# splinterhq/libsplinter

Measured on AMD Instinct MI355X. Metric: KV set/get ops/sec + Nomic-768d embed vectors/sec at 1/2/4/8 MI355X, higher is better.
Workload: dtype bf16

## Files before the change

libsplinter_amd/csrc/hip/gemm384.hip:

```cpp
#include <hip/hip_runtime.h>
#include <cstdint>
#include <cstdlib>

#include "gemm_tile.hpp"
#include "nomic_api.h"

namespace {

typedef __bf16 bf16x8 __attribute__((ext_vector_type(8)));
typedef __bf16 bf16x2_t __attribute__((ext_vector_type(2)));
typedef float f32x4 __attribute__((ext_vector_type(4)));
typedef __attribute__((address_space(3))) void lds_void;
typedef const __attribute__((address_space(1))) void gbl_void;

constexpr int kBM = spl::kGemm384BM;
constexpr int kBN = spl::kGemm384BN;
constexpr int kBK = 32;
constexpr int kWN = kBN / 2;
constexpr int kNT = kWN / 16;
constexpr int kThreads = 512;
constexpr int kRowBytes = kBK * 2;
constexpr int kABytes = kBM * kRowBytes;
constexpr int kWBytes = kBN * kRowBytes;

__device__ __forceinline__ uint32_t pk2(float a, float b) {
  const bf16x2_t v = {(__bf16)a, (__bf16)b};
  return __builtin_bit_cast(uint32_t, v);
}

__device__ __forceinline__ void raw_barrier() {
  asm volatile("" ::: "memory");
  __builtin_amdgcn_s_barrier();
  asm volatile("" ::: "memory");
}

__device__ __forceinline__ void wait_vm(int n) {
  switch (n) {
    case 3: asm volatile("s_waitcnt vmcnt(3)" ::: "memory"); break;
    default: asm volatile("s_waitcnt vmcnt(0)" ::: "memory"); break;
  }
}

__device__ __forceinline__ uint32_t xor16(uint32_t v) { return (uint32_t)__builtin_amdgcn_ds_swizzle((int)v, 0x401F); }

__device__ __forceinline__ int swz(int r, int c) { return c ^ ((r >> 1) & 3); }

__device__ __forceinline__ void rotate(float a, float b, float c, float s, bool plain, float& x1, float& x2) {
  float p1, p2;
  {
#pragma clang fp contract(off)
    p1 = a * c - b * s;
    p2 = b * c + a * s;
  }
  float bs, as;
  {
#pragma clang fp contract(off)
    bs = b * s;
    as = a * s;
  }
  const float f1 = __builtin_fmaf(a, c, -bs), f2 = __builtin_fmaf(b, c, as);
  x1 = plain ? p1 : f1;
  x2 = plain ? p2 : f2;
}

struct Epi384 {
  uint16_t* out;
  long ldo;
  const float* rope;
  const int32_t* pos;
  int rope_cols;
  long M;
  int gn;
};

constexpr int kNW = 3, kNA = 2;
constexpr int kLdsBytes = kNW * kWBytes + kNA * kABytes;
static_assert(kLdsBytes <= 160 * 1024, "LDS budget");

template <int MODE>
__global__ __launch_bounds__(kThreads, 1) void k_gemm384(const uint16_t* __restrict__ A, long lda,
                                                         const uint16_t* __restrict__ W, long ldw, int K,
                                                         int mtiles, int ntiles, Epi384 ep) {
  constexpr int LW = kNW - 1, LA = kNA - 1;
  static_assert(LW > LA, "an iteration issues its A stage before its W stage");
  constexpr int kABase = kNW * kWBytes;
  constexpr int kWaves = kThreads / 64;
  constexpr int RW = kBM / 4, MT = RW / 16;
  constexpr int GA = kBM / 16 / kWaves, GW = kBN / 16 / kWaves;
  static_assert(GA == 2 && GW == 3 && MT == 4, "wait_vm's cases and the epilogues assume this split");
  static_assert(MODE == NOMIC_EPI_STORE || MODE == NOMIC_EPI_SWIGLU || MODE == NOMIC_EPI_ROPE, "epilogues");
  extern __shared__ __attribute__((aligned(16))) char smem[];
  const int tid = threadIdx.x, lane = tid & 63, wave = tid >> 6;
  const int wr = wave >> 1, wn = wave & 1;
  int mt, nt;
  spl::remap_tile(blockIdx.x, mtiles * ntiles, ntiles, ep.gn, mt, nt);
  const long m0 = (long)mt * kBM, n0 = (long)nt * kBN;
  A += m0 * lda;
  W += n0 * ldw;

  const int drow = lane >> 2, dpc = lane & 3;
  uint32_t offA[GA];
#pragma unroll
  for (int i = 0; i < GA; ++i) {
    const int r = (wave + kWaves * i) * 16 + drow;
    const long gr = (m0 + r < ep.M) ? r : ep.M - 1 - m0;
    offA[i] = (uint32_t)(gr * lda + swz(r, dpc) * 8);
  }
  uint32_t offW[GW];
#pragma unroll
  for (int i = 0; i < GW; ++i) {
    const int r = (wave + kWaves * i) * 16 + drow;
    offW[i] = (uint32_t)(r * ldw + swz(r, dpc) * 8);
  }
  const int nk = K / kBK;
  auto glds_w = [&](int t, int i) {
    __builtin_amdgcn_global_load_lds((gbl_void*)(W + (long)t * kBK + offW[i]),
                                     (lds_void*)(smem + (t % kNW) * kWBytes + (wave + kWaves * i) * 1024), 16, 0, 0);
  };
  auto glds_a = [&](int t, int i) {
    __builtin_amdgcn_global_load_lds((gbl_void*)(A + (long)t * kBK + offA[i]),
                                     (lds_void*)(smem + kABase + (t % kNA) * kABytes + (wave + kWaves * i) * 1024),
                                     16, 0, 0);
  };
  constexpr int kOps = GA + GW;
  static_assert(kOps <= kNT, "two DMAs ahead of each of the kNT / 2 MFMA pairs cover a stage's loads");
  auto issue_op = [&](int s, int u) {
    const int tw = s + LW, ta = s + LA;
    if (u < GA) { if (ta >= 0 && ta < nk) glds_a(ta, u); }
    else if (tw >= 0 && tw < nk) glds_w(tw, u - GA);
  };
  auto issue = [&](int s) {
#pragma unroll
    for (int u = 0; u < kOps; ++u) issue_op(s, u);
  };
  auto younger = [&](int t) -> int { return t + LW - 1 < nk ? GW : 0; };

  const int fl = (lane & 15) * kRowBytes + (swz(lane & 15, lane >> 4) << 4);
  const int aoff = kABase + (wr * RW) * kRowBytes + fl;
  const int woff = (wn * kWN) * kRowBytes + fl;

  f32x4 acc[MT][kNT];
#pragma unroll
  for (int i = 0; i < MT; ++i)
#pragma unroll
    for (int j = 0; j < kNT; ++j) acc[i][j] = f32x4{0.f, 0.f, 0.f, 0.f};
  for (int s = -LW; s < 0; ++s) issue(s);
  for (int t = 0; t < nk; ++t) {
    wait_vm(younger(t));
    raw_barrier();
    const char* bw = smem + (t % kNW) * kWBytes;
    const char* ba = smem + (t % kNA) * kABytes;
    bf16x8 af[MT], w0, w1, x0, x1;
#pragma unroll
    for (int i = 0; i < MT; ++i) af[i] = *(const bf16x8*)(ba + aoff + i * 16 * kRowBytes);
    w0 = *(const bf16x8*)(bw + woff);
    w1 = *(const bf16x8*)(bw + woff + 16 * kRowBytes);
    __builtin_amdgcn_s_setprio(1);
#pragma unroll
    for (int jp = 0; jp < kNT / 2; ++jp) {
#pragma unroll
      for (int u = 2 * jp; u < 2 * jp + 2; ++u)
        if (u < kOps) issue_op(t, u);
      if (jp + 1 < kNT / 2) {
        x0 = *(const bf16x8*)(bw + woff + (2 * (jp + 1)) * 16 * kRowBytes);
        x1 = *(const bf16x8*)(bw + woff + (2 * (jp + 1) + 1) * 16 * kRowBytes);
      }
#pragma unroll
      for (int i = 0; i < MT; ++i) {
        acc[i][2 * jp] = __builtin_amdgcn_mfma_f32_16x16x32_bf16(w0, af[i], acc[i][2 * jp], 0, 0, 0);
        acc[i][2 * jp + 1] = __builtin_amdgcn_mfma_f32_16x16x32_bf16(w1, af[i], acc[i][2 * jp + 1], 0, 0, 0);
      }
      __builtin_amdgcn_sched_barrier(0);
      w0 = x0;
      w1 = x1;
    }
    __builtin_amdgcn_s_setprio(0);
  }

  const int rl = lane & 15, cq = (lane >> 4) * 4;
  const bool odd = (lane >> 4) & 1;
  const int h8 = (lane >> 5) * 8;
  const long mb = m0 + wr * RW + rl;
  auto exchange = [&](const uint32_t (&x)[2], const uint32_t (&y)[2]) -> uint4 {
    const uint32_t gx = xor16(odd ? x[0] : y[0]), gy = xor16(odd ? x[1] : y[1]);
    return odd ? make_uint4(gx, gy, y[0], y[1]) : make_uint4(x[0], x[1], gx, gy);
  };
  if constexpr (MODE == NOMIC_EPI_STORE) {
    uint16_t* o = ep.out + n0 + wn * kWN + (odd ? 16 : 0) + h8;
#pragma unroll
    for (int p = 0; p < kNT / 2; ++p)
#pragma unroll
      for (int i = 0; i < MT; ++i) {
        const long m = mb + 16 * i;
        const uint32_t x[2] = {pk2(acc[i][2 * p][0], acc[i][2 * p][1]), pk2(acc[i][2 * p][2], acc[i][2 * p][3])};
        const uint32_t y[2] = {pk2(acc[i][2 * p + 1][0], acc[i][2 * p + 1][1]),
                               pk2(acc[i][2 * p + 1][2], acc[i][2 * p + 1][3])};
        const uint4 v = exchange(x, y);
        if (m < ep.M) *(uint4*)(o + m * ep.ldo + 32 * p) = v;
      }
  } else if constexpr (MODE == NOMIC_EPI_SWIGLU) {
    uint16_t* o = ep.out + (n0 + wn * kWN) / 2 + (odd ? 16 : 0) + h8;
#pragma unroll
    for (int q = 0; q < kNT / 4; ++q)
#pragma unroll
      for (int i = 0; i < MT; ++i) {
        const long m = mb + 16 * i;
        uint32_t hk[2][2];
#pragma unroll
        for (int h = 0; h < 2; ++h) {
          const int p = 2 * q + h;
          float v[4];
#pragma unroll
          for (int e = 0; e < 4; ++e) v[e] = spl::swiglu(acc[i][2 * p][e], acc[i][2 * p + 1][e]);
          hk[h][0] = pk2(v[0], v[1]);
          hk[h][1] = pk2(v[2], v[3]);
        }
        const uint4 v = exchange(hk[0], hk[1]);
        if (m < ep.M) *(uint4*)(o + m * ep.ldo + 32 * q) = v;
      }
  } else {
#pragma unroll
    for (int i = 0; i < MT; ++i) {
      const long m = mb + 16 * i;
      const long mr = m < ep.M ? m : ep.M - 1;
      const bool rot = n0 + wn * kWN < ep.rope_cols;
      const float* cs0 = ep.rope + (rot ? (long)ep.pos[mr] * 64 : 0) + cq * 2;
#pragma unroll
      for (int half = 0; half < 2; ++half) {
        float4 ca = {}, cb = {};
        if (rot) ca = *(const float4*)(cs0 + half * 32), cb = *(const float4*)(cs0 + half * 32 + 4);
        const float cs[8] = {ca.x, ca.y, ca.z, ca.w, cb.x, cb.y, cb.z, cb.w};
#pragma unroll
        for (int head = 0; head < kWN / 64; ++head) {
          const int p = 2 * head + half;
          const long gcol = n0 + wn * kWN + head * 64;
          float x1[4], x2[4];
#pragma unroll
          for (int e = 0; e < 4; ++e) {
            x1[e] = acc[i][2 * p][e];
            x2[e] = acc[i][2 * p + 1][e];
          }
          if (gcol < ep.rope_cols) {
#pragma unroll
            for (int e = 0; e < 4; ++e) {
              rotate(x1[e], x2[e], cs[2 * e], cs[2 * e + 1], e >= 2 && odd, x1[e], x2[e]);
            }
          }
          const uint32_t x[2] = {pk2(x1[0], x1[1]), pk2(x1[2], x1[3])};
          const uint32_t y[2] = {pk2(x2[0], x2[1]), pk2(x2[2], x2[3])};
          const uint4 v = exchange(x, y);
          if (m < ep.M) *(uint4*)(ep.out + m * ep.ldo + gcol + (odd ? 32 : 0) + half * 16 + h8) = v;
        }
      }
    }
  }
}

template <int MODE>
int launch384(const uint16_t* A, long lda, const uint16_t* W, long ldw, long M, int N, int K, const Epi384& ep,
              hipStream_t s) {
  static bool attr = [] {
    (void)hipFuncSetAttribute((const void*)k_gemm384<MODE>, hipFuncAttributeMaxDynamicSharedMemorySize, kLdsBytes);
    return true;
  }();
  (void)attr;
  const int mtiles = (int)((M + kBM - 1) / kBM), ntiles = N / kBN;
  hipLaunchKernelGGL(k_gemm384<MODE>, dim3(mtiles * ntiles), dim3(kThreads), kLdsBytes, s, A, lda, W, ldw, K, mtiles,
                     ntiles, ep);
  return (int)hipGetLastError();
}

}

namespace spl {

bool gemm384_ok(int mode, const void* out, long ldo, long lda, long ldw, long M, int N, int K, const float* rope) {
  if (mode != NOMIC_EPI_STORE && mode != NOMIC_EPI_SWIGLU && mode != NOMIC_EPI_ROPE) return false;
  if (M <= 0 || N <= 0 || N % kBN || K % kBK || K < 2 * kBK) return false;
  if (lda % 8 || ldw % 8 || ldo % 8 || (uintptr_t)out % 16 || lda < K || ldw < K) return false;
  if (mode == NOMIC_EPI_ROPE && (uintptr_t)rope % 16) return false;
  const long mtiles = (M + kBM - 1) / kBM;
  return (long)kBM * lda < (1L << 31) && (long)kBN * ldw < (1L << 31) && mtiles * (N / kBN) < (1L << 31);
}

int gemm384_launch(int mode, const uint16_t* A, long lda, const uint16_t* W, long ldw, long M, int N, int K,
                   uint16_t* out, long ldo, const float* rope, const int32_t* pos, int rope_cols, int gn,
                   hipStream_t s) {
  const Epi384 ep{out, ldo, rope, pos, rope_cols, M, gn};
  switch (mode) {
    case NOMIC_EPI_STORE: return launch384<NOMIC_EPI_STORE>(A, lda, W, ldw, M, N, K, ep, s);
    case NOMIC_EPI_SWIGLU: return launch384<NOMIC_EPI_SWIGLU>(A, lda, W, ldw, M, N, K, ep, s);
    case NOMIC_EPI_ROPE: return launch384<NOMIC_EPI_ROPE>(A, lda, W, ldw, M, N, K, ep, s);
    default: return (int)hipErrorInvalidValue;
  }
}

}
```

libsplinter_amd/csrc/include/nomic_api.h:

```cpp
#ifndef SPLINTER_NOMIC_API_H
#define SPLINTER_NOMIC_API_H
#include <stdint.h>
#include "arena_api.h"

#ifdef __cplusplus
extern "C" {
#endif

#define NOMIC_EPI_STORE    0
#define NOMIC_EPI_RESIDUAL 1
#define NOMIC_EPI_SWIGLU   2
#define NOMIC_EPI_ROPE     3
#define NOMIC_EPI_F32      4
#define NOMIC_EPI_ROPE_FOLD    5
#define NOMIC_EPI_SWIGLU_FOLD  6
#define NOMIC_EPI_RES_STATS    7
#define NOMIC_EPI_RES_LN_STATS 8

int nomic_gemm(int mode, const void *A, long lda, const void *W, long ldw, long M, int N, int K,
               void *out, long ldo, const void *res, long ldr, const float *rope, const int32_t *pos,
               int rope_cols, hipStream_t stream);
int nomic_gemm_ln(int mode, const void *A, long lda, const void *W, long ldw, long M, int N, int K, void *out,
                  long ldo, const void *res, long ldr, const float *rope, const int32_t *pos, int rope_cols,
                  const float *part_in, int nparts, float eps, const float *c1, const float *c2,
                  const void *ln_g, const void *ln_b, float *part, hipStream_t stream);
int nomic_row_stats(const float *part, int nparts, long M, float eps, float *st, hipStream_t stream);
int nomic_gemm_set_variant(int variant);
int nomic_gemm_set_tail_split(int on);
long nomic_gemm256_grid(long M, int N);

int nomic_embed_ln(const int32_t *ids, long T, const void *tok_emb, const void *type_row,
                   const void *gamma, const void *beta, float eps, void *out, hipStream_t stream);
int nomic_layernorm(const void *x, long T, const void *gamma, const void *beta, float eps, void *out,
                    hipStream_t stream);
int nomic_attention_set_variant(int variant);
int nomic_attention(const void *qkv, void *out, const int32_t *cu_seqlens, const int32_t *qblocks,
                    int nqb, int heads, float scale, hipStream_t stream);
int nomic_mean_pool(const void *x, const int32_t *cu_seqlens, int B, float *pooled, int normalize,
                    spl_arena_t arena, const int64_t *slots, const uint64_t *hashes, int32_t *status,
                    hipStream_t stream);
int nomic_dequant(int ggml_type, const void *src, long nelems, void *dst_bf16, hipStream_t stream);

#ifdef __cplusplus
}
#endif
#endif
```

libsplinter_amd/models/nomic.py:

```python
from __future__ import annotations

import ctypes
import math
import os
from dataclasses import dataclass
from typing import Dict, List, Optional, Sequence, Tuple

import numpy as np
import torch

from .. import _native as N
from ..utils.tracing import trace_range
from .gguf import DEVICE_DEQUANT, GGUFFile, GGUFWriter, dequant_host

EPI_STORE, EPI_RESIDUAL, EPI_SWIGLU, EPI_ROPE, EPI_F32 = 0, 1, 2, 3, 4
EPI_ROPE_FOLD, EPI_SWIGLU_FOLD, EPI_RES_STATS, EPI_RES_LN_STATS = 5, 6, 7, 8


@dataclass
class NomicConfig:
    vocab: int = 30528
    d: int = 768
    layers: int = 12
    heads: int = 12
    ffn: int = 3072
    eps: float = 1e-12
    rope_base: float = 1000.0
    n_ctx: int = 2048
    type_vocab: int = 2

    @property
    def head_dim(self) -> int:
        return self.d // self.heads

    @classmethod
    def from_gguf(cls, g: GGUFFile) -> "NomicConfig":
        a = g.arch() or "nomic-bert"
        get = lambda k, d: g.get(f"{a}.{k}", d)
        tok = g.tensors.get("token_embd.weight")
        return cls(vocab=tok.shape[0] if tok else 30528, d=int(get("embedding_length", 768)),
                   layers=int(get("block_count", 12)), heads=int(get("attention.head_count", 12)),
                   ffn=int(get("feed_forward_length", 3072)), eps=float(get("attention.layer_norm_epsilon", 1e-12)),
                   rope_base=float(get("rope.freq_base", 1000.0)), n_ctx=int(get("context_length", 2048)))


def _lib():
    L = N.hip_lib()
    if not getattr(L, "_nomic_declared", False):
        P, c_long, c_int, c_float = ctypes.c_void_p, ctypes.c_long, ctypes.c_int, ctypes.c_float
        L.nomic_gemm.argtypes = [c_int, P, c_long, P, c_long, c_long, c_int, c_int, P, c_long, P, c_long, P, P, c_int, P]
        L.nomic_gemm.restype = c_int
        L.nomic_gemm_ln.argtypes = [c_int, P, c_long, P, c_long, c_long, c_int, c_int, P, c_long, P, c_long, P, P,
                                    c_int, P, c_int, c_float, P, P, P, P, P, P]
        L.nomic_gemm_ln.restype = c_int
        L.nomic_gemm_res_ln.argtypes = [P, c_long, P, c_long, c_long, c_int, c_int, P, c_long, P, P, c_float, P,
                                        c_long, P]
        L.nomic_gemm_res_ln.restype = c_int
        L.nomic_gemm_res_ln_set_variant.argtypes = [c_int]
        L.nomic_gemm_res_ln_set_variant.restype = c_int
        L.nomic_row_stats.argtypes = [P, c_int, c_long, c_float, P, P]
        L.nomic_row_stats.restype = c_int
        L.nomic_gemm_set_variant.argtypes = [c_int]
        L.nomic_gemm_set_variant.restype = c_int
        L.nomic_gemm_set_tail_split.argtypes = [c_int]
        L.nomic_gemm_set_tail_split.restype = c_int
        L.nomic_gemm256_grid.argtypes = [c_long, c_int]
        L.nomic_gemm256_grid.restype = c_long
        L.nomic_attention_set_variant.argtypes = [c_int]
        L.nomic_attention_set_variant.restype = c_int
        L.nomic_embed_ln.argtypes = [P, c_long, P, P, P, P, c_float, P, P]
        L.nomic_embed_ln.restype = c_int
        L.nomic_layernorm.argtypes = [P, c_long, P, P, c_float, P, P]
        L.nomic_layernorm.restype = c_int
        L.nomic_attention.argtypes = [P, P, P, P, c_int, c_int, c_float, P]
        L.nomic_attention.restype = c_int
        L.nomic_mean_pool.argtypes = [P, P, c_int, P, c_int, N.Arena, P, P, P, P]
        L.nomic_mean_pool.restype = c_int
        L.nomic_dequant.argtypes = [c_int, P, c_long, P, P]
        L.nomic_dequant.restype = c_int
        L._nomic_declared = True
    return L


def _chk(rc, what):
    if rc != 0:
        raise RuntimeError(f"{what}: HIP launch failed ({rc})")


def _stream():
    return torch.cuda.current_stream().cuda_stream


GGUF_NAMES = {
    "tok": "token_embd.weight", "type": "token_types.weight",
    "emb_g": "token_embd_norm.weight", "emb_b": "token_embd_norm.bias",
}
LAYER_NAMES = {
    "wqkv": "attn_qkv.weight", "wo": "attn_output.weight",
    "ln1_g": "attn_output_norm.weight", "ln1_b": "attn_output_norm.bias",
    "wup": "ffn_up.weight", "wgate": "ffn_gate.weight", "wdown": "ffn_down.weight",
    "ln2_g": "layer_output_norm.weight", "ln2_b": "layer_output_norm.bias",
}


def random_weights(cfg: NomicConfig, seed: int = 0, std: float = 0.02) -> Dict[str, np.ndarray]:
    rng = np.random.default_rng(seed)
    f = lambda *s: (rng.standard_normal(s) * std).astype(np.float32)
    w = {GGUF_NAMES["tok"]: f(cfg.vocab, cfg.d), GGUF_NAMES["type"]: f(cfg.type_vocab, cfg.d),
         GGUF_NAMES["emb_g"]: (1 + f(cfg.d) * 5).astype(np.float32), GGUF_NAMES["emb_b"]: f(cfg.d)}
    for i in range(cfg.layers):
        p = f"blk.{i}."
        w[p + "attn_qkv.weight"] = f(3 * cfg.d, cfg.d)
        w[p + "attn_output.weight"] = f(cfg.d, cfg.d)
        w[p + "attn_output_norm.weight"] = (1 + f(cfg.d) * 5).astype(np.float32)
        w[p + "attn_output_norm.bias"] = f(cfg.d)
        w[p + "ffn_up.weight"] = f(cfg.ffn, cfg.d)
        w[p + "ffn_gate.weight"] = f(cfg.ffn, cfg.d)
        w[p + "ffn_down.weight"] = f(cfg.d, cfg.ffn)
        w[p + "layer_output_norm.weight"] = (1 + f(cfg.d) * 5).astype(np.float32)
        w[p + "layer_output_norm.bias"] = f(cfg.d)
    return w


def write_gguf(path: str, cfg: NomicConfig, weights: Dict[str, np.ndarray], vocab: Optional[List[str]] = None,
               linear_type: str = "F16") -> None:
    w = GGUFWriter(path, "nomic-bert")
    a = "nomic-bert"
    w.add("general.name", "nomic-embed-text-v1.5 (random init)")
    w.add(f"{a}.context_length", cfg.n_ctx)
    w.add(f"{a}.embedding_length", cfg.d)
    w.add(f"{a}.feed_forward_length", cfg.ffn)
    w.add(f"{a}.attention.head_count", cfg.heads)
    w.add(f"{a}.attention.layer_norm_epsilon", float(cfg.eps))
    w.add(f"{a}.block_count", cfg.layers)
    w.add(f"{a}.rope.freq_base", float(cfg.rope_base))
    w.add(f"{a}.attention.causal", False)
    w.add(f"{a}.pooling_type", 1)
    if vocab is not None:
        w.add("tokenizer.ggml.model", "bert")
        w.add("tokenizer.ggml.tokens", vocab)
        w.add("tokenizer.ggml.token_type", [1] * len(vocab))
        ids = {t: i for i, t in enumerate(vocab)}
        for key, tok in (("bos", "[CLS]"), ("eos", "[SEP]"), ("seperator", "[SEP]"), ("unknown", "[UNK]"),
                         ("padding", "[PAD]")):
            if tok in ids:
                w.add(f"tokenizer.ggml.{key}_token_id", ids[tok])
    for name, arr in weights.items():
        lin = arr.ndim == 2 and not name.startswith("token_")
        w.add_tensor(name, arr, linear_type if lin else ("F16" if name == "token_embd.weight" else "F32"))
    w.write()


def pack_upgate(up: torch.Tensor, gate: torch.Tensor) -> torch.Tensor:
    F, d = up.shape
    return torch.stack([up.reshape(F // 16, 16, d), gate.reshape(F // 16, 16, d)], 1).reshape(2 * F, d)


_QKV_PERM = torch.cat([torch.arange(0, 16), torch.arange(32, 48), torch.arange(16, 32), torch.arange(48, 64)])


def pack_qkv(w: torch.Tensor) -> torch.Tensor:
    n, d = w.shape
    return w.reshape(n // 64, 64, d)[:, _QKV_PERM.to(w.device)].reshape(n, d)


def fold_ln(w: torch.Tensor, g: torch.Tensor, b: torch.Tensor):
    wf = (w.float() * g.float()[None, :]).to(torch.bfloat16).contiguous()
    c1 = wf.float().sum(1).contiguous()
    c2 = (w.float() @ b.float()).contiguous()
    return wf, c1, c2


class NomicWeights:

    def __init__(self, cfg: NomicConfig, tensors: Dict[str, torch.Tensor], device="cuda"):
        self.cfg = cfg
        bf = lambda t: t.to(device=device, dtype=torch.bfloat16).contiguous()
        self.tok = bf(tensors[GGUF_NAMES["tok"]])
        self.type_row = bf(tensors[GGUF_NAMES["type"]][0])
        self.emb_g, self.emb_b = bf(tensors[GGUF_NAMES["emb_g"]]), bf(tensors[GGUF_NAMES["emb_b"]])
        self.layers = []
        for i in range(cfg.layers):
            p = f"blk.{i}."
            t = {k: tensors[p + v] for k, v in LAYER_NAMES.items()}
            self.layers.append({
                "wqkv": bf(pack_qkv(t["wqkv"])), "wo": bf(t["wo"]), "wupgate": bf(pack_upgate(t["wup"], t["wgate"])),
                "wdown": bf(t["wdown"]),
                "ln1_g": bf(t["ln1_g"]), "ln1_b": bf(t["ln1_b"]), "ln2_g": bf(t["ln2_g"]), "ln2_b": bf(t["ln2_b"]),
            })
        for i, lw in enumerate(self.layers):
            lw["wupgate_f"], lw["ug_c1"], lw["ug_c2"] = fold_ln(lw["wupgate"], lw["ln1_g"], lw["ln1_b"])
            if i > 0:
                prev = self.layers[i - 1]
                lw["wqkv_f"], lw["qkv_c1"], lw["qkv_c2"] = fold_ln(lw["wqkv"], prev["ln2_g"], prev["ln2_b"])

    @classmethod
    def from_numpy(cls, cfg, weights: Dict[str, np.ndarray], device="cuda"):
        return cls(cfg, {k: torch.from_numpy(v) for k, v in weights.items()}, device)

    @classmethod
    def from_gguf(cls, g: GGUFFile, cfg: Optional[NomicConfig] = None, device="cuda"):
        cfg = cfg or NomicConfig.from_gguf(g)
        L = _lib()
        out = {}
        for name, info in g.tensors.items():
            if info.ggml_type in DEVICE_DEQUANT:
                raw = torch.from_numpy(np.ascontiguousarray(g.raw(name))).to(device)
                dst = torch.empty(info.nelems, dtype=torch.bfloat16, device=device)
                _chk(L.nomic_dequant(info.ggml_type, raw.data_ptr(), info.nelems, dst.data_ptr(), _stream()),
                     f"dequant {name}")
                out[name] = dst.view(info.shape)
            else:
                out[name] = torch.from_numpy(dequant_host(g.raw(name), info.ggml_type, info.nelems)
                                             .reshape(info.shape)).to(device)
        return cls(cfg, out, device)


class NomicReference(torch.nn.Module):

    def __init__(self, cfg: NomicConfig, weights: Dict[str, np.ndarray], device="cpu"):
        super().__init__()
        self.cfg = cfg
        self.w = {k: torch.from_numpy(np.asarray(v, np.float32)).to(device) for k, v in weights.items()}

    def rope(self, x, pos):
        hd = self.cfg.head_dim
        inv = self.cfg.rope_base ** (-torch.arange(0, hd, 2, dtype=torch.float64, device=x.device) / hd)
        ang = pos[:, None].double() * inv[None, :]
        c, s = torch.cos(ang).float()[:, None, :], torch.sin(ang).float()[:, None, :]
        x1, x2 = x[..., : hd // 2], x[..., hd // 2:]
        return torch.cat([x1 * c - x2 * s, x2 * c + x1 * s], dim=-1)

    def forward(self, ids: torch.Tensor, cu: Sequence[int]) -> torch.Tensor:
        cfg, w = self.cfg, self.w
        F = torch.nn.functional
        x = w["token_embd.weight"][ids] + w["token_types.weight"][0]
        x = F.layer_norm(x, (cfg.d,), w["token_embd_norm.weight"], w["token_embd_norm.bias"], cfg.eps)
        pos = torch.cat([torch.arange(cu[i + 1] - cu[i]) for i in range(len(cu) - 1)]).to(ids.device)
        H, hd = cfg.heads, cfg.head_dim
        for i in range(cfg.layers):
            p = f"blk.{i}."
            qkv = x @ w[p + "attn_qkv.weight"].T
            q, k, v = qkv.split(cfg.d, dim=1)
            q = self.rope(q.view(-1, H, hd), pos)
            k = self.rope(k.view(-1, H, hd), pos)
            v = v.view(-1, H, hd)
            outs = []
            for s in range(len(cu) - 1):
                a, b = cu[s], cu[s + 1]
                att = torch.einsum("qhd,khd->hqk", q[a:b], k[a:b]) / math.sqrt(hd)
                outs.append(torch.einsum("hqk,khd->qhd", att.softmax(-1), v[a:b]))
            o = torch.cat(outs).reshape(-1, cfg.d)
            x = F.layer_norm(o @ w[p + "attn_output.weight"].T + x, (cfg.d,), w[p + "attn_output_norm.weight"],
                             w[p + "attn_output_norm.bias"], cfg.eps)
            up = x @ w[p + "ffn_up.weight"].T
            gate = x @ w[p + "ffn_gate.weight"].T
            h = (up * F.silu(gate)) @ w[p + "ffn_down.weight"].T
            x = F.layer_norm(h + x, (cfg.d,), w[p + "layer_output_norm.weight"], w[p + "layer_output_norm.bias"],
                             cfg.eps)
        return torch.stack([x[cu[s]: cu[s + 1]].mean(0) for s in range(len(cu) - 1)])


class Batch:

    def __init__(self, seqs: Sequence[Sequence[int]], device="cuda", qblock: int = 128):
        lens = [len(s) for s in seqs]
        assert all(n > 0 for n in lens), "empty sequence"
        self.B = len(seqs)
        self.T = sum(lens)
        self.T_pad = (self.T + 127) // 128 * 128
        self.cu_host = np.concatenate([[0], np.cumsum(lens)]).astype(np.int32)
        self.max_len = max(lens)
        ids = np.zeros(self.T_pad, np.int32)
        ids[: self.T] = np.concatenate([np.asarray(s, np.int32) for s in seqs])
        pos = np.zeros(self.T_pad, np.int32)
        pos[: self.T] = np.concatenate([np.arange(n, dtype=np.int32) for n in lens])
        qb = np.asarray([(i, q0) for i, n in enumerate(lens) for q0 in range(0, n, qblock)], np.int32).reshape(-1)
        self.nqb = qb.size // 2
        self._ids_host, self._device, self._qblock, self._parts = ids, device, qblock, {}
        if str(device) == "cpu":
            self.ids, self.pos = torch.from_numpy(ids), torch.from_numpy(pos)
            self.cu, self.qblocks = torch.from_numpy(self.cu_host), torch.from_numpy(qb)
            return
        parts = (ids, pos, self.cu_host, qb)
        span = [(p.size + 3) // 4 * 4 for p in parts]
        host = torch.empty(sum(span), dtype=torch.int32, pin_memory=True)
        hv = host.numpy()
        o = 0
        for p, n in zip(parts, span):
            hv[o: o + p.size] = p
            o += n
        dev = host.to(device, non_blocking=True)
        o = 0
        views = []
        for p, n in zip(parts, span):
            views.append(dev[o: o + p.size])
            o += n
        self.ids, self.pos, self.cu, self.qblocks = views

    def split(self, parts: int):
        if parts in self._parts:
            return self._parts[parts]
        lens = np.diff(self.cu_host)
        cum = np.cumsum(lens)
        cuts = [0] + [int(np.searchsorted(cum, self.T * j / parts, side="left")) + 1 for j in range(1, parts)] + [self.B]
        out = []
        for j in range(parts):
            d0, d1 = cuts[j], cuts[j + 1]
            if d1 <= d0:
                continue
            r0, r1 = int(self.cu_host[d0]), int(self.cu_host[d1])
            seqs = [self._ids_host[self.cu_host[d]: self.cu_host[d + 1]].tolist() for d in range(d0, d1)]
            out.append((Batch(seqs, self._device, self._qblock), r0))
        self._parts[parts] = out
        return out


class NomicEncoder:

    def __init__(self, weights: NomicWeights, max_tokens: int = 1 << 17):
        self._split_streams = None
        self.w = weights
        self.cfg = weights.cfg
        self.L = _lib()
        cfg = self.cfg
        npos = max(cfg.n_ctx, 8192)
        inv = cfg.rope_base ** (-np.arange(0, cfg.head_dim, 2, dtype=np.float64) / cfg.head_dim)
        ang = np.arange(npos, dtype=np.float64)[:, None] * inv[None, :]
        tab = np.stack([np.cos(ang), np.sin(ang)], axis=-1).astype(np.float32)
        self.rope = torch.from_numpy(tab.reshape(npos, -1)).cuda()
        self._ws_tokens = 0
        self._ensure(max_tokens)

    def _ensure(self, T_pad: int):
        if T_pad <= self._ws_tokens:
            return
        cfg = self.cfg
        e = dict(dtype=torch.bfloat16, device="cuda")
        self.x = torch.empty((T_pad, cfg.d), **e)
        self.h = torch.empty((T_pad, cfg.d), **e)
        self.attn = torch.empty((T_pad, cfg.d), **e)
        self.qkv = torch.empty((T_pad, 3 * cfg.d), **e)
        self.ffn = torch.empty((T_pad, cfg.ffn), **e)
        self.h2 = torch.empty((T_pad, cfg.d), **e)
        f = dict(dtype=torch.float32, device="cuda")
        self.part1 = torch.empty((T_pad, 2 * (cfg.d // 128)), **f)
        self.part2 = torch.empty((T_pad, 2 * (cfg.d // 128)), **f)
        self._ws_tokens = T_pad

    def _gemm(self, mode, A, W, M, out, res=None, pos=None):
        N_, K = W.shape
        _chk(self.L.nomic_gemm(mode, A.data_ptr(), A.stride(0), W.data_ptr(), W.stride(0), M,
                               N_, K, out.data_ptr(), out.stride(0), res.data_ptr() if res is not None else None,
                               res.stride(0) if res is not None else 0, self.rope.data_ptr(),
                               pos.data_ptr() if pos is not None else None, 2 * self.cfg.d, _stream()), "gemm")

    def _gemm_ln(self, mode, A, W, M, out, res=None, pos=None, pin=None, c1=None, c2=None, ln=None, part=None):
        N_, K = W.shape
        ptr = lambda t: t.data_ptr() if t is not None else None
        _chk(self.L.nomic_gemm_ln(mode, A.data_ptr(), A.stride(0), W.data_ptr(), W.stride(0), M, N_, K,
                                  out.data_ptr(), out.stride(0), ptr(res), res.stride(0) if res is not None else 0,
                                  self.rope.data_ptr(), ptr(pos), 2 * self.cfg.d, ptr(pin),
                                  pin.shape[1] // 2 if pin is not None else 0, self.cfg.eps, ptr(c1), ptr(c2),
                                  ptr(ln[0]) if ln else None, ptr(ln[1]) if ln else None, ptr(part), _stream()),
             f"gemm_ln({mode})")

    schedule = os.environ.get("NOMIC_SCHEDULE", "folded" if os.environ.get("NOMIC_LN_FOLD", "0") != "0" else "fused")

    split_parts = int(os.environ.get("NOMIC_SPLIT", "1"))

    def hidden(self, b: Batch) -> torch.Tensor:
        if self.split_parts > 1 and self.schedule == "fused" and b.B >= 2 * self.split_parts:
            return self._hidden_split(b, self.split_parts)
        if self.schedule == "folded":
            return self._hidden_folded(b)
        if self.schedule == "split":
            return self._hidden_unfused(b)
        if self.schedule != "fused":
            raise ValueError(f"unknown encoder schedule {self.schedule!r}")
        return self._hidden_fused(b)

    def _res_ln(self, A, W, M, x, g, beta):
        N_, K = W.shape
        _chk(self.L.nomic_gemm_res_ln(A.data_ptr(), A.stride(0), W.data_ptr(), W.stride(0), M, N_, K, x.data_ptr(),
                                      x.stride(0), g.data_ptr(), beta.data_ptr(), self.cfg.eps, x.data_ptr(),
                                      x.stride(0), _stream()), "gemm_res_ln")

    def _hidden_fused(self, b: Batch) -> torch.Tensor:
        cfg, L, w = self.cfg, self.L, self.w
        assert b.max_len <= self.rope.shape[0]
        self._ensure(b.T_pad)
        s = _stream()
        T = b.T
        x, attn, qkv, ffn = self.x, self.attn, self.qkv, self.ffn
        _chk(L.nomic_embed_ln(b.ids.data_ptr(), T, w.tok.data_ptr(), w.type_row.data_ptr(), w.emb_g.data_ptr(),
                              w.emb_b.data_ptr(), cfg.eps, x.data_ptr(), s), "embed_ln")
        scale = 1.0 / math.sqrt(cfg.head_dim)
        for lw in w.layers:
            self._gemm(EPI_ROPE, x, lw["wqkv"], T, qkv, pos=b.pos)
            _chk(L.nomic_attention(qkv.data_ptr(), attn.data_ptr(), b.cu.data_ptr(), b.qblocks.data_ptr(), b.nqb,
                                   cfg.heads, scale, s), "attention")
            self._res_ln(attn, lw["wo"], T, x, lw["ln1_g"], lw["ln1_b"])
            self._gemm(EPI_SWIGLU, x, lw["wupgate"], T, ffn)
            self._res_ln(ffn, lw["wdown"], T, x, lw["ln2_g"], lw["ln2_b"])
        return x[:T]

    def _hidden_split(self, b: Batch, parts: int) -> torch.Tensor:
        cfg, L, w = self.cfg, self.L, self.w
        assert b.max_len <= self.rope.shape[0]
        self._ensure(b.T_pad)
        subs = b.split(parts)
        if self._split_streams is None or len(self._split_streams) < len(subs):
            self._split_streams = [torch.cuda.Stream() for _ in subs]
        cur = torch.cuda.current_stream()
        streams = self._split_streams[: len(subs)]
        for st in streams:
            st.wait_stream(cur)
        scale = 1.0 / math.sqrt(cfg.head_dim)
        views = []
        for (sb, r0), st in zip(subs, streams):
            views.append((sb, st, self.x[r0:], self.attn[r0:], self.qkv[r0:], self.ffn[r0:]))
        for sb, st, x, attn, qkv, ffn in views:
            with torch.cuda.stream(st):
                _chk(L.nomic_embed_ln(sb.ids.data_ptr(), sb.T, w.tok.data_ptr(), w.type_row.data_ptr(),
                                      w.emb_g.data_ptr(), w.emb_b.data_ptr(), cfg.eps, x.data_ptr(), st.cuda_stream),
                     "embed_ln")
        for lw in w.layers:
            for sb, st, x, attn, qkv, ffn in views:
                with torch.cuda.stream(st):
                    s_ = st.cuda_stream
                    T = sb.T
                    self._gemm(EPI_ROPE, x, lw["wqkv"], T, qkv, pos=sb.pos)
                    _chk(L.nomic_attention(qkv.data_ptr(), attn.data_ptr(), sb.cu.data_ptr(), sb.qblocks.data_ptr(),
                                           sb.nqb, cfg.heads, scale, s_), "attention")
                    self._res_ln(attn, lw["wo"], T, x, lw["ln1_g"], lw["ln1_b"])
                    self._gemm(EPI_SWIGLU, x, lw["wupgate"], T, ffn)
                    self._res_ln(ffn, lw["wdown"], T, x, lw["ln2_g"], lw["ln2_b"])
        for st in streams:
            cur.wait_stream(st)
        return self.x[: b.T]

    def _hidden_folded(self, b: Batch) -> torch.Tensor:
        cfg, L, w = self.cfg, self.L, self.w
        assert b.max_len <= self.rope.shape[0]
        self._ensure(b.T_pad)
        s = _stream()
        T = b.T
        x, h1, h2, attn, qkv, ffn = self.x, self.h, self.h2, self.attn, self.qkv, self.ffn
        p1, p2 = self.part1, self.part2
        _chk(L.nomic_embed_ln(b.ids.data_ptr(), T, w.tok.data_ptr(), w.type_row.data_ptr(), w.emb_g.data_ptr(),
                              w.emb_b.data_ptr(), cfg.eps, x.data_ptr(), s), "embed_ln")
        scale = 1.0 / math.sqrt(cfg.head_dim)
        prev = None
        for lw in w.layers:
            if prev is None:
                self._gemm(EPI_ROPE, x, lw["wqkv"], T, qkv, pos=b.pos)
            else:
                self._gemm_ln(EPI_ROPE_FOLD, h2, lw["wqkv_f"], T, qkv, pos=b.pos, pin=p2, c1=lw["qkv_c1"],
                              c2=lw["qkv_c2"])
            _chk(L.nomic_attention(qkv.data_ptr(), attn.data_ptr(), b.cu.data_ptr(), b.qblocks.data_ptr(), b.nqb,
                                   cfg.heads, scale, s), "attention")
            if prev is None:
                self._gemm_ln(EPI_RES_STATS, attn, lw["wo"], T, h1, res=x, part=p1)
            else:
                self._gemm_ln(EPI_RES_LN_STATS, attn, lw["wo"], T, h1, res=h2, pin=p2,
                              ln=(prev["ln2_g"], prev["ln2_b"]), part=p1)
            self._gemm_ln(EPI_SWIGLU_FOLD, h1, lw["wupgate_f"], T, ffn, pin=p1, c1=lw["ug_c1"], c2=lw["ug_c2"])
            self._gemm_ln(EPI_RES_LN_STATS, ffn, lw["wdown"], T, h2, res=h1, pin=p1, ln=(lw["ln1_g"], lw["ln1_b"]),
                          part=p2)
            prev = lw
        _chk(L.nomic_layernorm(h2.data_ptr(), T, prev["ln2_g"].data_ptr(), prev["ln2_b"].data_ptr(), cfg.eps,
                               x.data_ptr(), s), "ln_final")
        return x[:T]

    def _hidden_unfused(self, b: Batch) -> torch.Tensor:
        cfg, L, w = self.cfg, self.L, self.w
        assert b.max_len <= self.rope.shape[0]
        self._ensure(b.T_pad)
        s = _stream()
        T = b.T
        x, h, attn, qkv, ffn = self.x, self.h, self.attn, self.qkv, self.ffn
        _chk(L.nomic_embed_ln(b.ids.data_ptr(), T, w.tok.data_ptr(), w.type_row.data_ptr(), w.emb_g.data_ptr(),
                              w.emb_b.data_ptr(), cfg.eps, x.data_ptr(), s), "embed_ln")
        scale = 1.0 / math.sqrt(cfg.head_dim)
        for lw in w.layers:
            self._gemm(EPI_ROPE, x, lw["wqkv"], T, qkv, pos=b.pos)
            _chk(L.nomic_attention(qkv.data_ptr(), attn.data_ptr(), b.cu.data_ptr(), b.qblocks.data_ptr(), b.nqb,
                                   cfg.heads, scale, s), "attention")
            self._gemm(EPI_RESIDUAL, attn, lw["wo"], T, h, res=x)
            _chk(L.nomic_layernorm(h.data_ptr(), T, lw["ln1_g"].data_ptr(), lw["ln1_b"].data_ptr(), cfg.eps,
                                   x.data_ptr(), s), "ln1")
            self._gemm(EPI_SWIGLU, x, lw["wupgate"], T, ffn)
            self._gemm(EPI_RESIDUAL, ffn, lw["wdown"], T, h, res=x)
            _chk(L.nomic_layernorm(h.data_ptr(), T, lw["ln2_g"].data_ptr(), lw["ln2_b"].data_ptr(), cfg.eps,
                                   x.data_ptr(), s), "ln2")
        return x[:T]

    def embed(self, b: Batch, normalize: bool = False, arena=None, slots: Optional[torch.Tensor] = None,
              hashes: Optional[torch.Tensor] = None, out: Optional[torch.Tensor] = None):
        with trace_range("nomic.encoder"):
            self.hidden(b)
        if out is None:
            out = torch.empty((b.B, self.cfg.d), dtype=torch.float32, device="cuda")
        status = None
        desc = N.Arena()
        if arena is not None:
            desc = arena.desc
            status = torch.empty(b.B, dtype=torch.int32, device="cuda")
        _chk(self.L.nomic_mean_pool(self.x.data_ptr(), b.cu.data_ptr(), b.B, out.data_ptr(), int(normalize), desc,
                                    slots.data_ptr() if slots is not None else None,
                                    hashes.data_ptr() if hashes is not None else None,
                                    status.data_ptr() if status is not None else None, _stream()), "mean_pool")
        return (out, status) if arena is not None else out

    def flops(self, b: Batch) -> float:
        cfg = self.cfg
        lin = 2 * b.T * cfg.d * (3 * cfg.d + cfg.d + 2 * cfg.ffn + cfg.ffn) * cfg.layers
        lens = np.diff(b.cu_host)
        att = 4 * float((lens.astype(np.float64) ** 2).sum()) * cfg.d * cfg.layers
        return lin + att


def smoke_embed(arena, keys: torch.Tensor) -> None:
    cfg = NomicConfig(layers=2)
    w = NomicWeights.from_numpy(cfg, random_weights(cfg, seed=1))
    enc = NomicEncoder(w, max_tokens=1024)
    n = min(4, keys.shape[0])
    rng = np.random.default_rng(0)
    b = Batch([rng.integers(0, cfg.vocab, size=7 + 5 * i).tolist() for i in range(n)])
    st, idx = arena.meta("find", keys[:n])
    from ..parallel.sharded import GpuShard
    hashes = GpuShard(arena).hash_keys(keys[:n])
    vec, status = enc.embed(b, arena=arena, slots=idx, hashes=hashes)
    torch.cuda.synchronize()
    assert (status == 0).all(), status
    st2, back = arena.get_embeddings(keys[:n])
    assert torch.equal(back, vec), "slot vectors differ from pooled output"
    assert torch.isfinite(vec).all()
```

Baseline: 1.409 billion.

## Add BK=64 double-buffered pipeline variant to gemm384 and make it default

Adds a second main-loop path to the 384-wide GEMM kernel in which each stage loads a 64-wide K slice into one of two combined A+W LDS slots with a 128-byte-row swizzle. This halves the number of K iterations and therefore the barriers and waits per tile. The price is a full vmcnt(0) wait each iteration in place of the staggered 3-stage W / 2-stage A prefetch, so less load latency is hidden. It becomes the default when K is divisible by 64, with an environment variable and a C API to fall back to BK=32.

```diff
diff --git a/libsplinter_amd/csrc/hip/gemm384.hip b/libsplinter_amd/csrc/hip/gemm384.hip
--- a/libsplinter_amd/csrc/hip/gemm384.hip
+++ b/libsplinter_amd/csrc/hip/gemm384.hip
@@ -77,7 +77,13 @@
 constexpr int kLdsBytes = kNW * kWBytes + kNA * kABytes;
 static_assert(kLdsBytes <= 160 * 1024, "LDS budget");
 
-template <int MODE>
+constexpr int kWBytes2 = kBN * 128, kABytes2 = kBM * 128;
+constexpr int kSlotBytes = kWBytes2 + kABytes2;
+constexpr int kLdsBytes2 = 2 * kSlotBytes;
+static_assert(kLdsBytes2 <= 160 * 1024, "LDS budget");
+__device__ __forceinline__ int swz128(int r, int c) { return c ^ ((r >> 1) & 7); }
+
+template <int MODE, int BK>
 __global__ __launch_bounds__(kThreads, 1) void k_gemm384(const uint16_t* __restrict__ A, long lda,
                                                          const uint16_t* __restrict__ W, long ldw, int K,
                                                          int mtiles, int ntiles, Epi384 ep) {
@@ -89,6 +95,7 @@
   constexpr int GA = kBM / 16 / kWaves, GW = kBN / 16 / kWaves;
   static_assert(GA == 2 && GW == 3 && MT == 4, "wait_vm's cases and the epilogues assume this split");
   static_assert(MODE == NOMIC_EPI_STORE || MODE == NOMIC_EPI_SWIGLU || MODE == NOMIC_EPI_ROPE, "epilogues");
+  static_assert(BK == 32 || BK == 64, "K per stage");
   extern __shared__ __attribute__((aligned(16))) char smem[];
   const int tid = threadIdx.x, lane = tid & 63, wave = tid >> 6;
   const int wr = wave >> 1, wn = wave & 1;
@@ -98,83 +105,149 @@
   A += m0 * lda;
   W += n0 * ldw;
 
-  const int drow = lane >> 2, dpc = lane & 3;
-  uint32_t offA[GA];
-#pragma unroll
-  for (int i = 0; i < GA; ++i) {
-    const int r = (wave + kWaves * i) * 16 + drow;
-    const long gr = (m0 + r < ep.M) ? r : ep.M - 1 - m0;
-    offA[i] = (uint32_t)(gr * lda + swz(r, dpc) * 8);
-  }
-  uint32_t offW[GW];
-#pragma unroll
-  for (int i = 0; i < GW; ++i) {
-    const int r = (wave + kWaves * i) * 16 + drow;
-    offW[i] = (uint32_t)(r * ldw + swz(r, dpc) * 8);
-  }
-  const int nk = K / kBK;
-  auto glds_w = [&](int t, int i) {
-    __builtin_amdgcn_global_load_lds((gbl_void*)(W + (long)t * kBK + offW[i]),
-                                     (lds_void*)(smem + (t % kNW) * kWBytes + (wave + kWaves * i) * 1024), 16, 0, 0);
-  };
-  auto glds_a = [&](int t, int i) {
-    __builtin_amdgcn_global_load_lds((gbl_void*)(A + (long)t * kBK + offA[i]),
-                                     (lds_void*)(smem + kABase + (t % kNA) * kABytes + (wave + kWaves * i) * 1024),
-                                     16, 0, 0);
-  };
-  constexpr int kOps = GA + GW;
-  static_assert(kOps <= kNT, "two DMAs ahead of each of the kNT / 2 MFMA pairs cover a stage's loads");
-  auto issue_op = [&](int s, int u) {
-    const int tw = s + LW, ta = s + LA;
-    if (u < GA) { if (ta >= 0 && ta < nk) glds_a(ta, u); }
-    else if (tw >= 0 && tw < nk) glds_w(tw, u - GA);
-  };
-  auto issue = [&](int s) {
-#pragma unroll
-    for (int u = 0; u < kOps; ++u) issue_op(s, u);
-  };
-  auto younger = [&](int t) -> int { return t + LW - 1 < nk ? GW : 0; };
-
-  const int fl = (lane & 15) * kRowBytes + (swz(lane & 15, lane >> 4) << 4);
-  const int aoff = kABase + (wr * RW) * kRowBytes + fl;
-  const int woff = (wn * kWN) * kRowBytes + fl;
-
   f32x4 acc[MT][kNT];
 #pragma unroll
   for (int i = 0; i < MT; ++i)
 #pragma unroll
     for (int j = 0; j < kNT; ++j) acc[i][j] = f32x4{0.f, 0.f, 0.f, 0.f};
-  for (int s = -LW; s < 0; ++s) issue(s);
-  for (int t = 0; t < nk; ++t) {
-    wait_vm(younger(t));
-    raw_barrier();
-    const char* bw = smem + (t % kNW) * kWBytes;
-    const char* ba = smem + (t % kNA) * kABytes;
-    bf16x8 af[MT], w0, w1, x0, x1;
-#pragma unroll
-    for (int i = 0; i < MT; ++i) af[i] = *(const bf16x8*)(ba + aoff + i * 16 * kRowBytes);
-    w0 = *(const bf16x8*)(bw + woff);
-    w1 = *(const bf16x8*)(bw + woff + 16 * kRowBytes);
-    __builtin_amdgcn_s_setprio(1);
-#pragma unroll
-    for (int jp = 0; jp < kNT / 2; ++jp) {
-#pragma unroll
-      for (int u = 2 * jp; u < 2 * jp + 2; ++u)
-        if (u < kOps) issue_op(t, u);
-      if (jp + 1 < kNT / 2) {
-        x0 = *(const bf16x8*)(bw + woff + (2 * (jp + 1)) * 16 * kRowBytes);
-        x1 = *(const bf16x8*)(bw + woff + (2 * (jp + 1) + 1) * 16 * kRowBytes);
-      }
-#pragma unroll
-      for (int i = 0; i < MT; ++i) {
-        acc[i][2 * jp] = __builtin_amdgcn_mfma_f32_16x16x32_bf16(w0, af[i], acc[i][2 * jp], 0, 0, 0);
-        acc[i][2 * jp + 1] = __builtin_amdgcn_mfma_f32_16x16x32_bf16(w1, af[i], acc[i][2 * jp + 1], 0, 0, 0);
-      }
-      __builtin_amdgcn_sched_barrier(0);
-      w0 = x0;
-      w1 = x1;
-    }
-    __builtin_amdgcn_s_setprio(0);
+  if constexpr (BK == 32) {
+    const int drow = lane >> 2, dpc = lane & 3;
+    uint32_t offA[GA];
+#pragma unroll
+    for (int i = 0; i < GA; ++i) {
+      const int r = (wave + kWaves * i) * 16 + drow;
+      const long gr = (m0 + r < ep.M) ? r : ep.M - 1 - m0;
+      offA[i] = (uint32_t)(gr * lda + swz(r, dpc) * 8);
+    }
+    uint32_t offW[GW];
+#pragma unroll
+    for (int i = 0; i < GW; ++i) {
+      const int r = (wave + kWaves * i) * 16 + drow;
+      offW[i] = (uint32_t)(r * ldw + swz(r, dpc) * 8);
+    }
+    const int nk = K / kBK;
+    auto glds_w = [&](int t, int i) {
+      __builtin_amdgcn_global_load_lds((gbl_void*)(W + (long)t * kBK + offW[i]),
+                                       (lds_void*)(smem + (t % kNW) * kWBytes + (wave + kWaves * i) * 1024), 16, 0, 0);
+    };
+    auto glds_a = [&](int t, int i) {
+      __builtin_amdgcn_global_load_lds((gbl_void*)(A + (long)t * kBK + offA[i]),
+                                       (lds_void*)(smem + kABase + (t % kNA) * kABytes + (wave + kWaves * i) * 1024),
+                                       16, 0, 0);
+    };
+    constexpr int kOps = GA + GW;
+    static_assert(kOps <= kNT, "two DMAs ahead of each of the kNT / 2 MFMA pairs cover a stage's loads");
+    auto issue_op = [&](int s, int u) {
+      const int tw = s + LW, ta = s + LA;
+      if (u < GA) { if (ta >= 0 && ta < nk) glds_a(ta, u); }
+      else if (tw >= 0 && tw < nk) glds_w(tw, u - GA);
+    };
+    auto issue = [&](int s) {
+#pragma unroll
+      for (int u = 0; u < kOps; ++u) issue_op(s, u);
+    };
+    auto younger = [&](int t) -> int { return t + LW - 1 < nk ? GW : 0; };
+
+    const int fl = (lane & 15) * kRowBytes + (swz(lane & 15, lane >> 4) << 4);
+    const int aoff = kABase + (wr * RW) * kRowBytes + fl;
+    const int woff = (wn * kWN) * kRowBytes + fl;
+
+    for (int s = -LW; s < 0; ++s) issue(s);
+    for (int t = 0; t < nk; ++t) {
+      wait_vm(younger(t));
+      raw_barrier();
+      const char* bw = smem + (t % kNW) * kWBytes;
+      const char* ba = smem + (t % kNA) * kABytes;
+      bf16x8 af[MT], w0, w1, x0, x1;
+#pragma unroll
+      for (int i = 0; i < MT; ++i) af[i] = *(const bf16x8*)(ba + aoff + i * 16 * kRowBytes);
+      w0 = *(const bf16x8*)(bw + woff);
+      w1 = *(const bf16x8*)(bw + woff + 16 * kRowBytes);
+      __builtin_amdgcn_s_setprio(1);
+#pragma unroll
+      for (int jp = 0; jp < kNT / 2; ++jp) {
+#pragma unroll
+        for (int u = 2 * jp; u < 2 * jp + 2; ++u)
+          if (u < kOps) issue_op(t, u);
+        if (jp + 1 < kNT / 2) {
+          x0 = *(const bf16x8*)(bw + woff + (2 * (jp + 1)) * 16 * kRowBytes);
+          x1 = *(const bf16x8*)(bw + woff + (2 * (jp + 1) + 1) * 16 * kRowBytes);
+        }
+#pragma unroll
+        for (int i = 0; i < MT; ++i) {
+          acc[i][2 * jp] = __builtin_amdgcn_mfma_f32_16x16x32_bf16(w0, af[i], acc[i][2 * jp], 0, 0, 0);
+          acc[i][2 * jp + 1] = __builtin_amdgcn_mfma_f32_16x16x32_bf16(w1, af[i], acc[i][2 * jp + 1], 0, 0, 0);
+        }
+        __builtin_amdgcn_sched_barrier(0);
+        w0 = x0;
+        w1 = x1;
+      }
+      __builtin_amdgcn_s_setprio(0);
+    }
+  } else {
+    constexpr int GA2 = kBM / 8 / kWaves, GW2 = kBN / 8 / kWaves, kOps2 = GA2 + GW2;
+    static_assert(kOps2 <= kNT, "two pieces ahead of each of the first MFMA pairs cover a stage's loads");
+    const int drow = lane >> 3, dpc = lane & 7;
+    const int dsw = swz128(wave * 8 + drow, dpc) * 8;
+    uint32_t offA[GA2];
+#pragma unroll
+    for (int i = 0; i < GA2; ++i) {
+      const int r = (wave + kWaves * i) * 8 + drow;
+      const long gr = (m0 + r < ep.M) ? r : ep.M - 1 - m0;
+      offA[i] = (uint32_t)(gr * lda + dsw);
+    }
+    const uint32_t offW = (uint32_t)((wave * 8 + drow) * ldw + dsw);
+    const int nk = K / 64;
+    auto issue_op = [&](int t, int u) {
+      char* slot = smem + (t & 1) * kSlotBytes;
+      if (u < GA2)
+        __builtin_amdgcn_global_load_lds((gbl_void*)(A + (long)t * 64 + offA[u]),
+                                         (lds_void*)(slot + kWBytes2 + (wave + kWaves * u) * 1024), 16, 0, 0);
+      else
+        __builtin_amdgcn_global_load_lds((gbl_void*)(W + (long)t * 64 + (long)(u - GA2) * (kWaves * 8) * ldw + offW),
+                                         (lds_void*)(slot + (wave + kWaves * (u - GA2)) * 1024), 16, 0, 0);
+    };
+    const int fl = (lane & 15) * 128 + (swz128(lane & 15, lane >> 4) << 4);
+    const int aoff = kWBytes2 + (wr * RW) * 128 + fl;
+    const int woff = (wn * kWN) * 128 + fl;
+
+#pragma unroll
+    for (int u = 0; u < kOps2; ++u) issue_op(0, u);
+    for (int t = 0; t < nk; ++t) {
+      asm volatile("s_waitcnt vmcnt(0)" ::: "memory");
+      raw_barrier();
+      const char* bw = smem + (t & 1) * kSlotBytes;
+      bf16x8 af[MT], w0, w1, x0, x1;
+#pragma unroll
+      for (int i = 0; i < MT; ++i) af[i] = *(const bf16x8*)(bw + aoff + i * 16 * 128);
+      w0 = *(const bf16x8*)(bw + woff);
+      w1 = *(const bf16x8*)(bw + woff + 16 * 128);
+      __builtin_amdgcn_s_setprio(1);
+#pragma unroll
+      for (int q = 0; q < kNT; ++q) {
+        const int jp = q % (kNT / 2);
+        if (t + 1 < nk) {
+#pragma unroll
+          for (int u = 2 * q; u < 2 * q + 2; ++u)
+            if (u < kOps2) issue_op(t + 1, u);
+        }
+        if (q + 1 < kNT) {
+          const int h1 = (q + 1) / (kNT / 2), j1 = (q + 1) % (kNT / 2);
+          x0 = *(const bf16x8*)(bw + (woff ^ (h1 * 64)) + (2 * j1) * 16 * 128);
+          x1 = *(const bf16x8*)(bw + (woff ^ (h1 * 64)) + (2 * j1 + 1) * 16 * 128);
+        }
+#pragma unroll
+        for (int i = 0; i < MT; ++i) {
+          acc[i][2 * jp] = __builtin_amdgcn_mfma_f32_16x16x32_bf16(w0, af[i], acc[i][2 * jp], 0, 0, 0);
+          acc[i][2 * jp + 1] = __builtin_amdgcn_mfma_f32_16x16x32_bf16(w1, af[i], acc[i][2 * jp + 1], 0, 0, 0);
+          if (q == kNT / 2 - 1) af[i] = *(const bf16x8*)(bw + (aoff ^ 64) + i * 16 * 128);
+        }
+        __builtin_amdgcn_sched_barrier(0);
+        w0 = x0;
+        w1 = x1;
+      }
+      __builtin_amdgcn_s_setprio(0);
+    }
   }
 
   const int rl = lane & 15, cq = (lane >> 4) * 4;
@@ -256,18 +329,35 @@
   }
 }
 
-template <int MODE>
-int launch384(const uint16_t* A, long lda, const uint16_t* W, long ldw, long M, int N, int K, const Epi384& ep,
+int g_bk = -1;
+int gemm384_bk() {
+  if (g_bk < 0) {
+    const char* e = getenv("NOMIC_GEMM384_BK");
+    g_bk = e && atoi(e) == 32 ? 32 : 64;
+  }
+  return g_bk;
+}
+
+template <int MODE, int BK>
+int launch384_bk(const uint16_t* A, long lda, const uint16_t* W, long ldw, long M, int N, int K, const Epi384& ep,
               hipStream_t s) {
+  constexpr int lds = BK == 64 ? kLdsBytes2 : kLdsBytes;
   static bool attr = [] {
-    (void)hipFuncSetAttribute((const void*)k_gemm384<MODE>, hipFuncAttributeMaxDynamicSharedMemorySize, kLdsBytes);
+    (void)hipFuncSetAttribute((const void*)k_gemm384<MODE, BK>, hipFuncAttributeMaxDynamicSharedMemorySize, lds);
     return true;
   }();
   (void)attr;
   const int mtiles = (int)((M + kBM - 1) / kBM), ntiles = N / kBN;
-  hipLaunchKernelGGL(k_gemm384<MODE>, dim3(mtiles * ntiles), dim3(kThreads), kLdsBytes, s, A, lda, W, ldw, K, mtiles,
+  hipLaunchKernelGGL((k_gemm384<MODE, BK>), dim3(mtiles * ntiles), dim3(kThreads), lds, s, A, lda, W, ldw, K, mtiles,
                      ntiles, ep);
   return (int)hipGetLastError();
+}
+
+template <int MODE>
+int launch384(const uint16_t* A, long lda, const uint16_t* W, long ldw, long M, int N, int K, const Epi384& ep,
+              hipStream_t s) {
+  if (gemm384_bk() == 64 && K % 64 == 0) return launch384_bk<MODE, 64>(A, lda, W, ldw, M, N, K, ep, s);
+  return launch384_bk<MODE, 32>(A, lda, W, ldw, M, N, K, ep, s);
 }
 
 }
@@ -296,3 +386,9 @@
 }
 
 }
+
+extern "C" int nomic_gemm384_set_bk(int bk) {
+  const int prev = gemm384_bk();
+  g_bk = bk == 32 ? 32 : 64;
+  return prev;
+}
diff --git a/libsplinter_amd/csrc/include/nomic_api.h b/libsplinter_amd/csrc/include/nomic_api.h
--- a/libsplinter_amd/csrc/include/nomic_api.h
+++ b/libsplinter_amd/csrc/include/nomic_api.h
@@ -26,6 +26,7 @@
                   const void *ln_g, const void *ln_b, float *part, hipStream_t stream);
 int nomic_row_stats(const float *part, int nparts, long M, float eps, float *st, hipStream_t stream);
 int nomic_gemm_set_variant(int variant);
+int nomic_gemm384_set_bk(int bk);
 int nomic_gemm_set_tail_split(int on);
 long nomic_gemm256_grid(long M, int N);
 
diff --git a/libsplinter_amd/models/nomic.py b/libsplinter_amd/models/nomic.py
--- a/libsplinter_amd/models/nomic.py
+++ b/libsplinter_amd/models/nomic.py
@@ -62,6 +62,8 @@
         L.nomic_row_stats.restype = c_int
         L.nomic_gemm_set_variant.argtypes = [c_int]
         L.nomic_gemm_set_variant.restype = c_int
+        L.nomic_gemm384_set_bk.argtypes = [c_int]
+        L.nomic_gemm384_set_bk.restype = c_int
         L.nomic_gemm_set_tail_split.argtypes = [c_int]
         L.nomic_gemm_set_tail_split.restype = c_int
         L.nomic_gemm256_grid.argtypes = [c_long, c_int]
```

After: 1.443 billion, median of 6. +2.4%, better.
